# Avielstein/GRASP_LAB_SALP

Hardware: AMD Instinct MI355X
Metric: env-steps/sec at 65536 parallel envs, 1/2/4/8 MI355X; % HBM roofline (higher is better)
Workload: dtype f64

## Files before the change

grasp_lab_salp_amd/_codeobj.py:

```python
import hashlib
import struct

BUNDLE_MAGIC = b"__CLANG_OFFLOAD_BUNDLE__"


def _code_objects(blob):
    pos = 0
    while True:
        b = blob.find(BUNDLE_MAGIC, pos)
        if b < 0:
            return
        pos = b + len(BUNDLE_MAGIC)
        (n,) = struct.unpack_from("<Q", blob, pos)
        p = pos + 8
        for _ in range(n):
            off, size, idlen = struct.unpack_from("<QQQ", blob, p)
            p += 24
            ident = blob[p:p + idlen].decode("ascii", "replace")
            p += idlen
            if "amdgcn" in ident and size > 0:
                co = blob[b + off:b + off + size]
                if co[:4] == b"\x7fELF":
                    yield ident, co


def _symbols(co):
    shoff, = struct.unpack_from("<Q", co, 0x28)
    shentsize, shnum, _ = struct.unpack_from("<HHH", co, 0x3A)
    secs = []
    for k in range(shnum):
        (_name, sh_type, _flags, addr, off, size, link, _info, _align,
         entsize) = struct.unpack_from("<IIQQQQIIQQ", co, shoff + k * shentsize)
        secs.append((sh_type, addr, off, size, link, entsize))
    out = {}
    for sh_type, _addr, off, size, link, entsize in secs:
        if sh_type != 2:
            continue
        stroff = secs[link][2]
        for j in range(size // entsize):
            st_name, _st_info, _st_other, shndx, value, ssize = struct.unpack_from("<IBBHQQ", co, off + j * entsize)
            if shndx == 0 or shndx >= len(secs) or ssize == 0:
                continue
            end = co.index(b"\0", stroff + st_name)
            name = co[stroff + st_name:end].decode("ascii", "replace")
            s_addr, s_off = secs[shndx][1], secs[shndx][2]
            out[name] = (value - s_addr + s_off, ssize)
    return out


def kernel_symbols(lib_path, contains):
    blob = open(lib_path, "rb").read()
    names = set()
    for _ident, co in _code_objects(blob):
        syms = _symbols(co)
        names |= {n for n in syms if contains in n and n + ".kd" in syms}
    return sorted(names)


def _mask_layout(code):
    n = len(code) // 4
    w = list(struct.unpack("<%dI" % n, code[:4 * n]))
    for i in range(n):
        if (w[i] & 0xFF80FFFF) != 0xBE801C00:
            continue
        j = i + 1
        while j + 1 < n and j <= i + 4:
            op = w[j] & 0xFF800000
            lit = (w[j] & 0xFF) == 0xFF or (w[j] >> 8 & 0xFF) == 0xFF
            if op in (0x80000000, 0x82000000) and lit:
                w[j + 1] = 0
                j += 2
            else:
                j += 1
    return struct.pack("<%dI" % n, *w) + code[4 * n:]


def kernel_sha(lib_path, contains):
    blob = open(lib_path, "rb").read()
    for _ident, co in _code_objects(blob):
        syms = _symbols(co)
        hits = [n for n in syms if contains in n and n + ".kd" in syms]
        if len(hits) == 1:
            symbol = hits[0]
            h = hashlib.sha256()
            off, size = syms[symbol]
            h.update(_mask_layout(co[off:off + size]))
            off, size = syms[symbol + ".kd"]
            kd = bytearray(co[off:off + size])
            kd[16:24] = bytes(8)
            h.update(bytes(kd))
            return h.hexdigest()[:16]
    return None


ROLLOUT_KERNEL = "k_rolloutILb0ELb0EE"
PAIR_COLLECT_KERNEL = "k_rollout_pairILb1EE"
SPLIT_COLLECT_KERNEL = "k_rollout_splitILb1EE"


def collect_kernel():
    import os
    if (os.environ.get("SALP_TWO_WAVE_KERNEL") or "").startswith("p"):
        return PAIR_COLLECT_KERNEL, "k_rollout_pair<true>"
    return SPLIT_COLLECT_KERNEL, "k_rollout_split<true>"
```

grasp_lab_salp_amd/build.py:

```python
import argparse
import os
import subprocess
import sys

HERE = os.path.dirname(os.path.abspath(__file__))
SRCS = [os.path.join(HERE, "csrc", f) for f in ("salp_kernels.hip", "salp_gae.hip", "salp_ppo.hip", "salp_ppo_mlp.hip",
                                               "salp_sort.hip", "salp_lstm.hip", "salp_sac.hip")]
OUT = os.path.join(HERE, "libsalp.so")
ARCH = os.environ.get("SALP_OFFLOAD_ARCH", "gfx950")
HIPCC = os.environ.get("HIPCC", "/opt/rocm/bin/hipcc")

FLAGS = ["-O3", "-std=c++17", f"--offload-arch={ARCH}", "-ffp-contract=off", "-fno-fast-math",
         "-fPIC", "-shared", "-Wall", "-Wno-unused-function"]


def deps():
    c = os.path.join(HERE, "csrc")
    return SRCS + [os.path.join(c, f) for f in os.listdir(c) if f.endswith(".h")] + [
        os.path.join(HERE, "..", "include", "salp.h")]


def up_to_date():
    if not os.path.exists(OUT):
        return False
    t = os.path.getmtime(OUT)
    return all(os.path.getmtime(d) <= t for d in deps())


FILE_FLAGS = {"salp_ppo_mlp.hip": ["-mllvm", "-amdgpu-sched-strategy=max-ilp"]}


def build(force=False, verbose=False, extra=(), out=None, file_flags=None):
    if out is None and not force and up_to_date():
        return OUT
    out = out or OUT
    file_flags = FILE_FLAGS if file_flags is None else file_flags
    import tempfile
    from concurrent.futures import ThreadPoolExecutor
    compile_flags = [f for f in FLAGS if f != "-shared"]
    with tempfile.TemporaryDirectory(prefix="salp_build_") as tmp:
        objs = [os.path.join(tmp, os.path.basename(src) + ".o") for src in SRCS]
        cmds = [[HIPCC, *compile_flags, *file_flags.get(os.path.basename(src), []), *extra, "-c", "-o", obj, src]
                for src, obj in zip(SRCS, objs)]
        link = [HIPCC, f"--offload-arch={ARCH}", "-fPIC", "-shared", "-o", out + ".tmp", *objs]
        if verbose:
            for c in cmds + [link]:
                print(" ".join(c), flush=True)
        with ThreadPoolExecutor(max_workers=min(len(cmds), os.cpu_count() or 1)) as ex:
            for r in list(ex.map(lambda c: subprocess.run(c, capture_output=True, text=True), cmds)):
                if r.returncode:
                    raise subprocess.CalledProcessError(r.returncode, r.args, r.stdout, r.stderr)
                if r.stderr and verbose:
                    print(r.stderr, end="", flush=True)
        subprocess.run(link, check=True)
    os.replace(out + ".tmp", out)
    return out


if __name__ == "__main__":
    ap = argparse.ArgumentParser()
    ap.add_argument("--verbose", action="store_true")
    ap.add_argument("--force", action="store_true")
    ap.add_argument("--resource-usage", action="store_true")
    a = ap.parse_args()
    extra = ["-Rpass-analysis=kernel-resource-usage"] if a.resource_usage else []
    print(build(force=a.force or a.resource_usage, verbose=a.verbose, extra=extra))
    sys.exit(0)
```

grasp_lab_salp_amd/csrc/salp_kernels.hip:

```cpp
#include <hip/hip_runtime.h>

#include <cmath>
#include <cstdio>
#include <cstdlib>
#include <cstring>
#include <string>

#include "salp_device.h"
#include "salp_pair.h"
#include "salp_tanh.h"

using salp::Hot;
using salp::Params;

#define SF(f) salp::sref(S, P, i, (f))

namespace {

constexpr int kBlock = 256;
constexpr int kMaxTicksPerCycle = 1 << 16;
constexpr int64_t kSortMinEnvs = 1024;

static_assert(kBlock == salp::LANES, "LDS cache stride is the workgroup size");

// ... 236 lines not shown
    }
    if (reward_sum) reward_sum[i] = rs;
    salp::store_hot<RAND>(h, S, P, i);
}

__global__ __launch_bounds__(kBlock) void k_predict_ticks(const double* S, Params P, const float* actions,
                                                          int32_t n_steps, uint32_t* keys, int32_t* ids) {
    const int64_t i = (int64_t)blockIdx.x * blockDim.x + threadIdx.x;
    if (i >= P.n) return;
    double a1 = SF(SALP_F_ANGLE1), a2 = SF(SALP_F_ANGLE2);
    int64_t t = 0;
    if (actions) {
        t = salp::predict_cycle_ticks(P, actions[3 * i], actions[3 * i + 1], actions[3 * i + 2], &a1, &a2);
    } else {
        const uint64_t env_id = (uint64_t)(P.env_offset + i), sc = (uint64_t)SF(SALP_F_STEP_COUNT);
        for (int32_t k = 0; k < n_steps; ++k) {
            float a[3];
            sp_action(P.seed, env_id, sc + (uint64_t)k, a);
            t += salp::predict_cycle_ticks(P, a[0], a[1], a[2], &a1, &a2);
        }
    }
    keys[i] = (uint32_t)(t > 65535 ? 65535 : t);
    ids[i] = (int32_t)i;
}

constexpr int kPH = SALP_POLICY_HIDDEN, kPIN = SALP_OBS_DIM_MAX;
typedef const __attribute__((address_space(4))) float* PolicyW;

typedef float PolicyF2 __attribute__((ext_vector_type(2)));
static_assert(kPH % 2 == 0, "hidden units go in pairs");

__device__ __forceinline__ float policy_tanh(float x) { return salp_tanhf(x); }

__device__ __forceinline__ void policy_layer1(PolicyW w, int w1, int b1, const float* x, float* h1) {
#pragma unroll
    for (int j = 0; j < kPH; j += 2) {
        PolicyF2 acc = {w[b1 + j], w[b1 + j + 1]};
#pragma unroll
        for (int k = 0; k < kPIN; ++k) {
            const PolicyF2 wk = {w[w1 + j * kPIN + k], w[w1 + (j + 1) * kPIN + k]};
            const PolicyF2 xk = {x[k], x[k]};
            acc = __builtin_elementwise_fma(wk, xk, acc);
        }
        h1[j] = policy_tanh(acc.x);
        h1[j + 1] = policy_tanh(acc.y);
    }
}

template <int NOUT>
__device__ __forceinline__ void policy_mlp(PolicyW w, int w1, int b1, int w2, int b2, int hw,
                                           int hb, const float* x, float* out) {
    float h1[kPH];
    policy_layer1(w, w1, b1, x, h1);
#pragma unroll
    for (int c = 0; c < NOUT; ++c) out[c] = 0.0f;
#pragma unroll 1
    for (int j = 0; j < kPH; ++j) {
        PolicyF2 acc = {w[b2 + j], 0.0f};
#pragma unroll
        for (int k = 0; k < kPH; k += 2) {
            const PolicyF2 wk = {w[w2 + j * kPH + k], w[w2 + j * kPH + k + 1]};
            const PolicyF2 hk = {h1[k], h1[k + 1]};
            acc = __builtin_elementwise_fma(wk, hk, acc);
        }
        const float t = policy_tanh(acc.x + acc.y);
#pragma unroll
        for (int c = 0; c < NOUT; ++c) out[c] = fmaf(w[hw + c * kPH + j], t, out[c]);
    }
#pragma unroll
    for (int c = 0; c < NOUT; ++c) out[c] += w[hb + c];
}

constexpr int kPolL2 = kPH * kPH + kPH + 3 * kPH;
static_assert(SALP_POLICY_PI_B2 == SALP_POLICY_PI_W2 + kPH * kPH && SALP_POLICY_ACT_W == SALP_POLICY_PI_B2 + kPH,
              "the staged actor tensors are contiguous in the packed policy");
__device__ __forceinline__ void policy_actor_l2(PolicyW w, const float* l2, const float* x, float* out) {
    float h1[kPH];
    policy_layer1(w, SALP_POLICY_PI_W1, SALP_POLICY_PI_B1, x, h1);
    out[0] = out[1] = out[2] = 0.0f;
#pragma unroll 1
    for (int j = 0; j < kPH; ++j) {
        const float* row = l2 + j * kPH;
        PolicyF2 acc = {l2[kPH * kPH + j], 0.0f};
#pragma unroll
        for (int k = 0; k < kPH; k += 4) {
            const float4 v = *reinterpret_cast<const float4*>(row + k);
            acc = __builtin_elementwise_fma(PolicyF2{v.x, v.y}, PolicyF2{h1[k], h1[k + 1]}, acc);
            acc = __builtin_elementwise_fma(PolicyF2{v.z, v.w}, PolicyF2{h1[k + 2], h1[k + 3]}, acc);
        }
        const float t = policy_tanh(acc.x + acc.y);
#pragma unroll
        for (int c = 0; c < 3; ++c) out[c] = fmaf(l2[kPH * kPH + kPH + c * kPH + j], t, out[c]);
    }
#pragma unroll
    for (int c = 0; c < 3; ++c) out[c] += w[SALP_POLICY_ACT_B + c];
}

__device__ __forceinline__ void policy_input(const float* o, int obs_dim, float* x) {
#pragma unroll
    for (int k = 0; k < kPIN; ++k) x[k] = k < obs_dim ? o[k] : 0.0f;
}

__device__ __forceinline__ float policy_value(PolicyW w, const float* x) {
    float v;
    policy_mlp<1>(w, SALP_POLICY_VF_W1, SALP_POLICY_VF_B1, SALP_POLICY_VF_W2, SALP_POLICY_VF_B2, SALP_POLICY_VAL_W,
                  SALP_POLICY_VAL_B, x, &v);
    return v;
}

#define SP_STREAM_POLICY 7u
__device__ __forceinline__ void policy_noise(uint64_t seed, uint64_t env_id, uint64_t step, float z[3]) {
    const sp_u32x4 r = sp_draw(seed, env_id, step, SP_STREAM_POLICY, 0);
    const double u1 = ((double)r.v[0] + 1.0) * 0x1.0p-32, u3 = ((double)r.v[2] + 1.0) * 0x1.0p-32;
    const double rad1 = sqrt(-2.0 * sm_log(u1)), rad2 = sqrt(-2.0 * sm_log(u3));
    double s1, c1, s2, c2;
    sm_sincos(6.283185307179586 * sp_u01_32(r.v[1]), &s1, &c1);
    sm_sincos(6.283185307179586 * sp_u01_32(r.v[3]), &s2, &c2);
    z[0] = (float)(rad1 * c1);
    z[1] = (float)(rad1 * s1);
    z[2] = (float)(rad2 * c2);
}

template <bool L2 = false>
__device__ __forceinline__ void policy_act(const SalpPolicyRollout& R, int obs_dim, const float* o, uint64_t env_id,
                                           uint64_t step, float a[3], float* value, float* logp,
                                           const float* l2 = nullptr) {
    const PolicyW w = (PolicyW)R.weights;
    float x[kPIN];
    policy_input(o, obs_dim, x);
    float mean[3];
    if (L2)
        policy_actor_l2(w, l2, x, mean);
    else
        policy_mlp<3>(w, SALP_POLICY_PI_W1, SALP_POLICY_PI_B1, SALP_POLICY_PI_W2, SALP_POLICY_PI_B2,
                      SALP_POLICY_ACT_W, SALP_POLICY_ACT_B, x, mean);
    if (value) *value = policy_value(w, x);
    float z[3];
    policy_noise(R.noise_seed, env_id, step, z);
    float lp = 0.0f;
#pragma unroll
    for (int c = 0; c < 3; ++c) {
        const float ls = w[SALP_POLICY_LOG_STD + c], sd = expf(ls);
        a[c] = mean[c] + sd * z[c];
        const float d = a[c] - mean[c];
        lp += -(d * d) / (2.0f * (sd * sd)) - logf(sd) - 0.91893853320467274f;
    }
    *logp = lp;
}

struct ValuesInPlace {
    static constexpr bool kDefer = false;
    static constexpr bool kL2 = false;
    __device__ __forceinline__ const float* l2() const { return nullptr; }
    __device__ __forceinline__ void start_rep() {}
    __device__ __forceinline__ void boot(const float*, int, float, int64_t) {}
    __device__ __forceinline__ void value(const float*, int, int64_t) {}
    __device__ __forceinline__ void publish() {}
};

#ifndef SALP_COLLECT_REP_MIN
#define SALP_COLLECT_REP_MIN 4
#endif

__device__ __forceinline__ float clamp_box(float a, float lo, float hi) { return a < lo ? lo : (a > hi ? hi : a); }

template <bool RAND, bool POL, class ST, class VS = ValuesInPlace>
__device__ __forceinline__ void rollout_boundary(Hot& h, ST S, const Params& P, int64_t i,
                                                 uint64_t env_id, bool& pending, bool& active,
                                                 int64_t& steps, int64_t max_steps,
                                                 const SalpRolloutBuffers& B, double* reward_sum,
                                                 const SalpPolicyRollout& R, salp::Cache32 c32, VS vs = VS()) {
    float o[SALP_OBS_DIM_MAX];
    bool have_o = false;
    float ep_start = 0.0f;
    for (int rep = 0; rep < 4; ++rep) {
        const bool fin = active && pending && !(h.ct < h.b2);
        vs.start_rep();
        if (fin) {
            SF(SALP_F_STEP_COUNT) = SF(SALP_F_STEP_COUNT) + 1.0;
            salp::StepOut r = salp::finish_step<RAND>(h, S, P, i, o, nullptr);
            bool reset = r.terminated || r.truncated;
            if (POL) {
                const size_t row = (size_t)steps * (size_t)P.n + (size_t)i;
                float rew = (float)r.reward;
                bool bad = false;
                if (R.diverged_obs_abs > 0.0) {
                    bad = !(fabs(r.reward) <= R.diverged_reward_abs);
                    for (int k = 0; k < P.obs_dim; ++k) bad = bad || !(fabsf(o[k]) <= (float)R.diverged_obs_abs);
                }
                if (bad) {
                    rew = 0.0f;
                    atomicAdd((unsigned long long*)R.diverged, 1ull);
                } else if (r.truncated && !r.terminated) {
                    if (VS::kDefer) {
                        vs.boot(o, P.obs_dim, rew, (int64_t)steps);
                    } else {
                        float x[kPIN];
                        policy_input(o, P.obs_dim, x);
                        rew = rew + (float)R.gamma * policy_value((PolicyW)R.weights, x);
                    }
                }
                if (reset && !bad) {
                    atomicAdd(&R.ep_stats[0], SF(SALP_F_EP_RETURN));
                    atomicAdd(&R.ep_stats[1], 1.0);
                    if (r.terminated) atomicAdd(&R.ep_stats[2], 1.0);
                    atomicAdd(&R.ep_stats[3], SF(SALP_F_EP_LEN));
                }
                if (!(VS::kDefer && !bad && r.truncated && !r.terminated)) R.rewards[row] = rew;
                reset = reset || bad;
                ep_start = reset ? 1.0f : 0.0f;
                R.episode_start[i] = ep_start;
            } else if (B.capacity > 0) {
                const size_t slot = (size_t)(steps % B.capacity);
                const size_t row = slot * (size_t)P.n + (size_t)i;
                if (B.obs)
                    for (int k = 0; k < P.obs_dim; ++k) B.obs[row * P.obs_dim + k] = o[k];
                if (B.actions) {
                    B.actions[row * 3 + 0] = (float)SF(SALP_F_ACT0);
                    B.actions[row * 3 + 1] = (float)SF(SALP_F_ACT1);
                    B.actions[row * 3 + 2] = (float)SF(SALP_F_ACT2);
                }
                if (B.rewards) B.rewards[row] = (float)r.reward;
                if (B.dones) B.dones[row] = (uint8_t)((r.terminated ? 1 : 0) | (r.truncated ? 2 : 0));
            }
            if (reward_sum) reward_sum[i] += r.reward;
            ++steps;
            pending = false;
            if (reset) salp::reset_env_philox(h, S, P, i, (POL || B.obs_before) ? o : nullptr);
            have_o = true;
            if (max_steps > 0 && steps >= max_steps) {
                active = false;
                if (POL)
                    for (int k = 0; k < P.obs_dim; ++k) R.last_obs[(size_t)i * P.obs_dim + k] = o[k];
            }
        }
        const bool beg = active && !pending;
        if (beg) {
            if (POL && !have_o) {
                for (int k = 0; k < P.obs_dim; ++k) o[k] = R.last_obs[(size_t)i * P.obs_dim + k];
                have_o = true;
            } else if (B.obs_before && !have_o) {
                const salp::Rot Rt = salp::rot_zyx(h.e0, h.e1, h.e2);
                salp::observation(h, Rt, S, P, i, o);
                have_o = true;
            }
            if (POL && VS::kDefer) vs.value(o, P.obs_dim, (int64_t)steps);
        }
        vs.publish();
        if (beg) {
            float a[3];
            if (POL) {
                if (!fin) ep_start = R.episode_start[i];
                float raw[3], v, lp;
                policy_act<VS::kL2>(R, P.obs_dim, o, env_id, (uint64_t)SF(SALP_F_STEP_COUNT), raw,
                                    VS::kDefer ? nullptr : &v, &lp, vs.l2());
                const size_t row = (size_t)steps * (size_t)P.n + (size_t)i;
                for (int k = 0; k < P.obs_dim; ++k) R.obs[row * P.obs_dim + k] = o[k];
                R.actions[row * 3 + 0] = raw[0];
                R.actions[row * 3 + 1] = raw[1];
                R.actions[row * 3 + 2] = raw[2];
                if (!VS::kDefer) R.values[row] = v;
                R.log_probs[row] = lp;
                R.episode_starts[row] = ep_start;
                a[0] = clamp_box(raw[0], 0.0f, 1.0f);
                a[1] = clamp_box(raw[1], 0.0f, 1.0f);
                a[2] = clamp_box(raw[2], -1.0f, 1.0f);
            } else {
                if (B.obs_before && B.capacity > 0) {
                    const size_t row = (size_t)(steps % B.capacity) * (size_t)P.n + (size_t)i;
                    for (int k = 0; k < P.obs_dim; ++k) B.obs_before[row * P.obs_dim + k] = o[k];
                }
                sp_action(P.seed, env_id, (uint64_t)SF(SALP_F_STEP_COUNT), a);
            }
            salp::begin_step<RAND>(h, S, P, i, a[0], a[1], a[2], c32);
            pending = true;
        }
        if (POL && SALP_COLLECT_REP_MIN > 1) {
            const bool again = active && pending && !(h.ct < h.b2);
            if (__popcll(__ballot(again)) < SALP_COLLECT_REP_MIN) break;
        }
        if (VS::kDefer) {
            if (!__any(fin || beg)) break;
        } else if (!fin && !beg) {
            break;
        }
    }
}

struct RolloutArgs {
    double* S;
    Params P;
    int64_t n_chunks;
    int32_t chunk;
    int32_t steady_q8;
    int64_t max_steps;
    SalpRolloutBuffers B;
    double* reward_sum;
    int32_t fresh;
    int32_t pad_;
    SalpPolicyRollout R;
};
static_assert(sizeof(RolloutArgs) % 8 == 0, "RolloutArgs is copied as 8-byte words");
typedef const __attribute__((address_space(4))) uint64_t* KernargWords;
__device__ __forceinline__ RolloutArgs fresh_args() {
    KernargWords p = (KernargWords)__builtin_amdgcn_kernarg_segment_ptr();
    asm volatile("" : "+s"(p));
    uint64_t w[sizeof(RolloutArgs) / 8];
    for (size_t k = 0; k < sizeof(RolloutArgs) / 8; ++k) w[k] = p[k];
    RolloutArgs a;
    __builtin_memcpy(&a, w, sizeof a);
    return a;
}

#ifndef SALP_ROLLOUT_RESEAT
#define SALP_ROLLOUT_RESEAT 1
#endif

__device__ __forceinline__ int nth_set_lane(const uint64_t* m, int k) {
    constexpr int NW = kBlock / 64;
    int base = 0;
    uint64_t w = m[NW - 1];
#pragma unroll
    for (int j = 0; j < NW - 1; ++j) {
        const int c = __popcll(m[j]);
        if (k < c) {
            w = m[j];
            base = 64 * j;
            break;
        }
        k -= c;
        base = 64 * (j + 1);
    }
    int pos = 0;
#pragma unroll
    for (int half = 32; half > 0; half >>= 1) {
        const uint64_t lo = w & ((1ull << half) - 1ull);
        const int c = __popcll(lo);
        if (k >= c) {
            k -= c;
            w >>= half;
            pos += half;
        } else {
            w = lo;
        }
    }
    return base + pos;
}

__device__ __forceinline__ bool unsteady(const Hot& h, const Params& P, bool active) {
    return active && h.ct < h.b2 && !salp::next_tick_steady(h, P);
}

template <bool RAND, bool POL>
__device__ __forceinline__ bool lane_boundary(const RolloutArgs& a, salp::SpillSlot sp, int64_t i, bool& pending,
                                              bool& active, int64_t& steps, double* c32p) {
    const uint64_t env_id = (uint64_t)(a.P.env_offset + i);
    salp::ColdRegs<RAND> C;
    salp::load_cold<RAND>(C, a.S, a.P, i);
    Hot hb;
    salp::unspill<RAND>(hb, sp, a.P, env_id);
    rollout_boundary<RAND, POL>(hb, &C, a.P, i, env_id, pending, active, steps, a.max_steps, a.B,
                                a.reward_sum, a.R, salp::Cache32{c32p});
    salp::store_cold<RAND>(C, a.S, a.P, i);
    salp::spill<RAND>(hb, sp);
    return unsteady(hb, a.P, active);
}
template <bool RAND, bool POL>
__device__ __noinline__ bool lane_boundary_call(const RolloutArgs* a, double* spp, int64_t i, bool* pending,
                                                bool* active, int64_t* steps, double* c32p) {
    return lane_boundary<RAND, POL>(*a, salp::SpillSlot{spp}, i, *pending, *active, *steps, c32p);
}

#ifndef SALP_ROLLOUT_PROF
#define SALP_ROLLOUT_PROF 0
#endif
enum { RP_BOUNDARY, RP_FULL, RP_STEADY, RP_SETTLED, RP_BARRIER, RP_RESEAT, RP_N };
__device__ unsigned long long g_roll_prof[2][RP_N];
struct RollProf {
    unsigned long long cyc[RP_N] = {}, its[RP_N] = {};
    unsigned long long t = 0;
    __device__ __forceinline__ void start() {
        if (SALP_ROLLOUT_PROF) t = __builtin_amdgcn_s_memtime();
    }
    __device__ __forceinline__ void lap(int part, int64_t iterations = 0) {
        if (SALP_ROLLOUT_PROF) {
            const unsigned long long now = __builtin_amdgcn_s_memtime();
            cyc[part] += now - t;
            its[part] += (unsigned long long)iterations;
            t = now;
        }
    }
    __device__ __forceinline__ void flush() {
        if (SALP_ROLLOUT_PROF && (threadIdx.x & 63) == 0)
            for (int k = 0; k < RP_N; ++k) {
                atomicAdd(&g_roll_prof[0][k], cyc[k]);
                atomicAdd(&g_roll_prof[1][k], its[k]);
            }
    }
};

#if SALP_ROLLOUT_RESEAT
template <bool RAND, bool POL>
__global__ __launch_bounds__(kBlock) void k_rollout(RolloutArgs A) {
    double* const S = A.S;
    const Params& P = A.P;
    const int64_t base = (int64_t)blockIdx.x * blockDim.x;
    const int lane = (int)threadIdx.x;
    __shared__ double s_cache32[salp::C32_N * salp::LANES];
    __shared__ double s_spill[salp::SPILL_N * salp::LANES];
    __shared__ int64_t s_steps[kBlock];
    __shared__ uint8_t s_flags[kBlock];
    __shared__ int16_t s_slot[2][kBlock];
    __shared__ uint64_t s_mask[2][kBlock / 64];
    __shared__ uint64_t s_amask[2][kBlock / 64];
    int s = lane;
    int64_t i = base + s;
    bool pending = false, active = false;
    int64_t steps = 0;
    Hot h{};
    if (i < P.n) {
        pending = !A.fresh && SF(SALP_F_PENDING) != 0.0;
        steps = A.B.steps_done ? A.B.steps_done[i] : 0;
        active = !(A.max_steps > 0 && steps >= A.max_steps);
        salp::load_hot<RAND>(h, S, P, i);
        salp::resume_cycle(h, S, P, i);
        salp::fill_cache32(P, h.c, salp::Cache32{s_cache32 + s});
    }
    if (!active) h.b2 = -INFINITY;
    bool all_done = false;
    RollProf prof;
    prof.start();
    for (int64_t c = 0;; ++c) {
        const bool last = c == A.n_chunks || all_done;
        const salp::SpillSlot sp{s_spill + s};
        const bool need = active && (!pending || !(h.ct < h.b2));
        bool uns = unsteady(h, P, active);
        salp::spill<RAND>(h, sp);
        if (need) {
            if (RAND) {
                uns = lane_boundary_call<RAND, POL>(&A, s_spill + s, i, &pending, &active, &steps, s_cache32 + s);
            } else {
                const RolloutArgs a = fresh_args();
                uns = lane_boundary<RAND, POL>(a, sp, i, pending, active, steps, s_cache32 + s);
            }
        }
        if (last) {
            const RolloutArgs a = fresh_args();
            salp::unspill<RAND>(h, sp, a.P, (uint64_t)(a.P.env_offset + i));
            if (i < a.P.n) salp::store_hot<RAND>(h, a.S, a.P, i);
            break;
        }
        const int b = (int)(c & 1);
        s_steps[s] = steps;
        s_flags[s] = (uint8_t)((pending ? 1 : 0) | (active ? 2 : 0));
        s_slot[b][lane] = (int16_t)s;
        const uint64_t ballot = __ballot(uns);
        const uint64_t aballot = __ballot(active);
        if ((lane & 63) == 0) {
            s_mask[b][lane >> 6] = ballot;
            s_amask[b][lane >> 6] = aballot;
        }
        prof.lap(RP_BOUNDARY);
        __syncthreads();
        prof.lap(RP_BARRIER);
        uint64_t m[kBlock / 64];
        int n_uns = 0;
        uint64_t any_active = 0;
#pragma unroll
        for (int w = 0; w < kBlock / 64; ++w) {
            m[w] = s_mask[b][w];
            n_uns += __popcll(m[w]);
            any_active |= s_amask[b][w];
        }
        all_done = any_active == 0;
        int from;
        if (lane < n_uns) {
            from = nth_set_lane(m, lane);
        } else {
#pragma unroll
            for (int w = 0; w < kBlock / 64; ++w) m[w] = ~m[w];
            from = nth_set_lane(m, lane - n_uns);
        }
        s = s_slot[b][from];
        i = base + s;
        const int fl = s_flags[s];
        pending = (fl & 1) != 0;
        active = (fl & 2) != 0;
        steps = s_steps[s];
        {
            const RolloutArgs a = fresh_args();
            salp::unspill<RAND>(h, salp::SpillSlot{s_spill + s}, a.P, (uint64_t)(a.P.env_offset + i));
        }
        if (!active) h.b2 = -INFINITY;
        if (all_done) continue;
        prof.lap(RP_RESEAT);
        const salp::Cache32 c32{s_cache32 + s};
        const Params PV = salp::pin_params(P);
        int32_t k = 0;
        for (; k < A.chunk; ++k) {
            if (__all(!(h.ct < h.b2) || salp::next_tick_steady(h, PV))) break;
            if (h.ct < h.b2) salp::tick<false, RAND, true>(h, PV, c32);
        }
        prof.lap(RP_FULL, k);
        const int32_t ks = (int32_t)(((int64_t)(A.chunk - k) * A.steady_q8) >> 8);
        int32_t j = 0;
        for (; j < ks; ++j) {
            bool settled = true;
            if (h.ct < h.b2) settled = salp::tick<false, RAND, true, true>(h, PV, c32);
            if (__all(settled)) {
                ++j;
                break;
            }
        }
        prof.lap(RP_STEADY, j);
        const int32_t j0 = j;
        for (; j < ks; ++j)
            if (h.ct < h.b2) salp::tick<false, RAND, true, true, true>(h, PV, c32);
        prof.lap(RP_SETTLED, j - j0);
    }
    prof.flush();
    if (A.B.steps_done && i < P.n) A.B.steps_done[i] = steps;
}
#else
template <bool RAND, bool POL>
__global__ __launch_bounds__(kBlock) void k_rollout(RolloutArgs A) {
    double* const S = A.S;
    const Params& P = A.P;
    int64_t i = (int64_t)blockIdx.x * blockDim.x + threadIdx.x;
    if (i >= P.n) return;
    bool pending = !A.fresh && SF(SALP_F_PENDING) != 0.0;
    int64_t steps = A.B.steps_done ? A.B.steps_done[i] : 0;
    bool active = !(A.max_steps > 0 && steps >= A.max_steps);
    LANE_CACHE32();
    __shared__ double s_spill[salp::SPILL_N * salp::LANES];
    const salp::SpillSlot sp{s_spill + threadIdx.x};
    Hot h;
    salp::load_hot<RAND>(h, S, P, i);
    salp::resume_cycle(h, S, P, i);
    salp::fill_cache32(P, h.c, c32);
    if (!active) h.b2 = -INFINITY;
    for (int64_t c = 0; c <= A.n_chunks; ++c) {
        const bool need = active && (!pending || !(h.ct < h.b2));
        const bool last = c == A.n_chunks || !__any(active || need);
        if (__any(need) || last) {
            salp::spill<RAND>(h, sp);
            if (need) {
                const RolloutArgs a = fresh_args();
                const uint64_t env_id = (uint64_t)(a.P.env_offset + i);
                salp::ColdRegs<RAND> C;
                salp::load_cold<RAND>(C, a.S, a.P, i);
                Hot hb;
                salp::unspill<RAND>(hb, sp, a.P, env_id);
                rollout_boundary<RAND, POL>(hb, &C, a.P, i, env_id, pending, active, steps, a.max_steps, a.B,
                                            a.reward_sum, a.R, c32);
                salp::store_cold<RAND>(C, a.S, a.P, i);
                salp::spill<RAND>(hb, sp);
            }
            {
                const RolloutArgs a = fresh_args();
                salp::unspill<RAND>(h, sp, a.P, (uint64_t)(a.P.env_offset + i));
                if (last) {
                    salp::store_hot<RAND>(h, a.S, a.P, i);
                    break;
                }
            }
            if (!active) h.b2 = -INFINITY;
        }
        const Params PV = salp::pin_params(P);
        for (int32_t k = 0; k < A.chunk; ++k)
            if (h.ct < h.b2) salp::tick<false, RAND, true>(h, PV, c32);
    }
    if (A.B.steps_done) A.B.steps_done[i] = steps;
}
#endif

constexpr int kPairEnvs = 128;
constexpr int kXchAB = 5;
constexpr int kXchBA = 13;
constexpr int kXchBase = 4 * kXchAB * 64;
constexpr int kXchDoubles = kXchBase + 4 * kXchBA * 64;
static_assert(kXchDoubles <= salp::SPILL_N * kPairEnvs, "the packets live in the spill slots' LDS");
constexpr int kPairSpin = 1 << 21;
__device__ unsigned int g_pair_timeouts;

#ifndef SALP_PAIR_PROF
#define SALP_PAIR_PROF 0
#endif
enum { PP_BOUNDARY, PP_TICK, PP_PUBLISH, PP_WAIT, PP_READ, PP_WORLD, PP_BARRIER, PP_N };
__device__ unsigned long long g_pair_prof[2][PP_N];
struct PairProf {
    unsigned long long acc[PP_N] = {};
    unsigned long long t = 0;
    __device__ __forceinline__ void start() {
        if (SALP_PAIR_PROF) t = __builtin_amdgcn_s_memtime();
    }
    __device__ __forceinline__ void lap(int phase) {
        if (SALP_PAIR_PROF) {
            const unsigned long long now = __builtin_amdgcn_s_memtime();
            acc[phase] += now - t;
            t = now;
        }
    }
    __device__ __forceinline__ void flush(int role) {
        if (SALP_PAIR_PROF && (threadIdx.x & 63) == 0)
            for (int k = 0; k < PP_N; ++k) atomicAdd(&g_pair_prof[role][k], acc[k]);
    }
};

struct PairShared {
    double cache32[salp::C32_N * kPairEnvs];
    double big[salp::SPILL_N * kPairEnvs];
    int64_t steps[kPairEnvs];
    int16_t slot[2][kPairEnvs];
    uint64_t mask[2][2], amask[2][2];
    int cnt[2][2];
    int mode[2][2];
    uint8_t flags[kPairEnvs];
};

struct PairJobs {
    __attribute__((aligned(16))) float pi_l2[kPolL2];
    float boot_obs[4][kPIN][kPairEnvs];
    float val_obs[4][kPIN][kPairEnvs];
    float boot_rew[4][kPairEnvs];
    int32_t boot_step[4][kPairEnvs];
    int32_t val_step[4][kPairEnvs];
    uint8_t flags[4][kPairEnvs];
    int cnt[2];
    int done[2];
};

__device__ __forceinline__ bool pair_wait(int* flag, int target) {
    for (int it = 0; it < kPairSpin; ++it) {
        if (__hip_atomic_load(flag, __ATOMIC_ACQUIRE, __HIP_MEMORY_SCOPE_WORKGROUP) >= target) return true;
        __builtin_amdgcn_s_sleep(1);
    }
    if ((threadIdx.x & 63) == 0) atomicAdd(&g_pair_timeouts, 1u);
    return false;
}
__device__ __forceinline__ void pair_publish(int* flag, int value) {
    __hip_atomic_store(flag, value, __ATOMIC_RELEASE, __HIP_MEMORY_SCOPE_WORKGROUP);
}

constexpr int kWaveRing = 64;
enum { WR_V0, WR_V1, WR_V2, WR_W0, WR_W1, WR_W2, WR_STRIDE = 6 };
enum { WX_E0, WX_E1, WX_E2, WX_P0, WX_P1, WX_P2, WX_SP, WX_CP, WX_ST, WX_CTH, WX_FAIL, WX_N };
struct WaveShared {
    double rows[kWave * WG_STRIDE];
    double ring[kWaveRing * WR_STRIDE];
    double xchg[WX_N];
    double c32[salp::C32_N];
    int produced, consumed;
};

template <bool RAND>
__device__ __forceinline__ bool run_cycle_split(Hot& h, const Params& P, salp::Cache32 c32, WaveShared& W) {
    const bool kin = threadIdx.x >= kWave;
    bool ok = true;
    int g = 0;
    if (!kin) {
        while (h.ct < h.b2 && g < kMaxTicksPerCycle) {
            wave_geometry_rows(h, P, c32, W.rows);
            __builtin_amdgcn_fence(__ATOMIC_ACQ_REL, "workgroup");
            int last = 0;
            for (int j = 0; j < kWave && h.ct < h.b2 && g < kMaxTicksPerCycle; ++j, ++g) {
                double x[WG_RI1 + 1];
                const double* r = W.rows + j * WG_STRIDE;
#pragma unroll
                for (int k = 0; k <= WG_RI1; ++k) x[k] = r[k];
                const bool settled = h.phase != salp::JET &&
                                     (__double_as_longlong(h.geo.mr) | __double_as_longlong(h.comr) |
                                      __double_as_longlong(h.coma)) == 0 &&
                                     h.geo.I0 == h.pI0 && h.geo.I1 == h.pI1 && h.pI2 == h.pI1;
                if (settled)
                    salp::tick_dynamics<false, RAND, true, salp::TD_FORCES | salp::TD_POSITIONS>(h, P, nullptr, 0);
                else
                    salp::tick_dynamics<false, RAND, false, salp::TD_FORCES | salp::TD_POSITIONS>(h, P, nullptr, 0);
                if (g >= kWaveRing) ok = pair_wait(&W.consumed, g - kWaveRing + 1) && ok;
                double* q = W.ring + (g % kWaveRing) * WR_STRIDE;
                q[WR_V0] = h.v0; q[WR_V1] = h.v1; q[WR_V2] = h.v2;
                q[WR_W0] = h.w0; q[WR_W1] = h.w1; q[WR_W2] = h.w2;
                pair_publish(&W.produced, g + 1);
                h.ct = x[WG_CT]; h.time = x[WG_TIME]; h.phase = (int)x[WG_PHASE]; h.W = x[WG_W];
                h.com = x[WG_COM]; h.comr = x[WG_COMR]; h.coma = x[WG_COMA];
                salp::Geo& q2 = h.geo;
                q2.m = x[WG_M]; q2.mr = x[WG_MR]; q2.I0 = x[WG_I0]; q2.I1 = x[WG_I1];
                q2.kc0 = x[WG_KC0]; q2.kc1 = x[WG_KC1]; q2.ra0 = x[WG_RA0]; q2.ra1 = x[WG_RA1];
                q2.dimx = x[WG_DIMX]; q2.dimy = x[WG_DIMY]; q2.speed = x[WG_SPEED]; q2.rx = x[WG_RX];
                q2.rm = x[WG_RM]; q2.rI0 = x[WG_RI0]; q2.rI1 = x[WG_RI1];
                last = j;
            }
            const double* r = W.rows + last * WG_STRIDE;
            h.L = r[WG_L]; h.V = r[WG_V]; h.pV = r[WG_PV];
            h.g32 = r[WG_G32] != 0.0; h.pv32 = r[WG_PV32] != 0.0;
            __builtin_amdgcn_fence(__ATOMIC_ACQ_REL, "workgroup");
        }
    } else {
        double ct = h.ct;
        for (; ct < h.b2 && g < kMaxTicksPerCycle; ++g) {
            ok = pair_wait(&W.produced, g + 1) && ok;
            const double* q = W.ring + (g % kWaveRing) * WR_STRIDE;
            h.v0 = q[WR_V0]; h.v1 = q[WR_V1]; h.v2 = q[WR_V2];
            h.w0 = q[WR_W0]; h.w1 = q[WR_W1]; h.w2 = q[WR_W2];
            pair_publish(&W.consumed, g + 1);
            salp::tick_dynamics<false, RAND, false, salp::TD_KINEMATICS>(h, P, nullptr, 0);
            ct += salp::DT;
        }
    }
    return ok;
}

template <bool RAND>
__global__ __launch_bounds__(2 * kWave) void k_step_wave(double* S, Params P, const float* actions,
                                                         float* obs_out, double* reward_out,
                                                         uint8_t* term_out, uint8_t* trunc_out,
                                                         int auto_reset, float* term_obs_out, double* info_out) {
    const int64_t i = blockIdx.x;
    if (i >= P.n) return;
    __shared__ __attribute__((aligned(16))) WaveShared W;
    const salp::Cache32 c32{W.c32, 1};
    const bool kin = threadIdx.x >= kWave;
    if (threadIdx.x == 0) {
        W.produced = 0;
        W.consumed = 0;
    }
    Hot h;
    salp::load_hot<RAND>(h, S, P, i);
    {
        salp::ColdRegs<RAND> C;
        salp::load_cold<RAND>(C, S, P, i);
        salp::begin_step<RAND>(h, &C, P, i, actions[3 * i], actions[3 * i + 1], actions[3 * i + 2], c32);
        if (!kin) salp::store_cold<RAND>(C, S, P, i);
    }
    __syncthreads();
    const bool ok = run_cycle_split<RAND>(h, P, c32, W);
    __syncthreads();
    if (kin) {
        if (threadIdx.x == kWave) {
            double* x = W.xchg;
            x[WX_E0] = h.e0; x[WX_E1] = h.e1; x[WX_E2] = h.e2;
            x[WX_P0] = h.p0; x[WX_P1] = h.p1; x[WX_P2] = h.p2;
            x[WX_SP] = h.sp; x[WX_CP] = h.cp; x[WX_ST] = h.st; x[WX_CTH] = h.cth;
            x[WX_FAIL] = ok ? 0.0 : 1.0;
        }
    }
    __syncthreads();
    if (kin) return;
    {
        const double* x = W.xchg;
        h.e0 = x[WX_E0]; h.e1 = x[WX_E1]; h.e2 = x[WX_E2];
        h.p0 = x[WX_P0]; h.p1 = x[WX_P1]; h.p2 = x[WX_P2];
        h.sp = x[WX_SP]; h.cp = x[WX_CP]; h.st = x[WX_ST]; h.cth = x[WX_CTH];
        if (!ok || x[WX_FAIL] != 0.0) salp::poison_motion(h);
    }
    float o[SALP_OBS_DIM_MAX];
    double* info = info_out ? info_out + (size_t)SALP_INFO_DIM * i : nullptr;
    salp::ColdRegs<RAND> C;
    salp::load_cold<RAND>(C, S, P, i);
    double& sc = salp::sref(&C, P, i, SALP_F_STEP_COUNT);
    sc = sc + 1.0;
    const salp::StepOut r = salp::finish_step<RAND>(h, &C, P, i, o, info);
    if (term_obs_out)
        for (int k = 0; k < P.obs_dim; ++k) term_obs_out[(size_t)i * P.obs_dim + k] = o[k];
    if (auto_reset && (r.terminated || r.truncated)) salp::reset_env_philox(h, &C, P, i, o);
    salp::store_cold<RAND>(C, S, P, i);
    if (reward_out) reward_out[i] = r.reward;
    if (term_out) term_out[i] = r.terminated;
    if (trunc_out) trunc_out[i] = r.truncated;
    if (obs_out)
        for (int k = 0; k < P.obs_dim; ++k) obs_out[(size_t)i * P.obs_dim + k] = o[k];
    salp::store_hot<RAND>(h, S, P, i);
}

struct ValuesToPartner {
    static constexpr bool kDefer = true;
    static constexpr bool kL2 = true;
    PairJobs* J;
    int grp, s, buf;
    __device__ __forceinline__ const float* l2() const { return J->pi_l2; }
    __device__ __forceinline__ void start_rep() {
        buf = __hip_atomic_load(&J->cnt[grp], __ATOMIC_RELAXED, __HIP_MEMORY_SCOPE_WORKGROUP) & 3;
    }
    __device__ __forceinline__ void boot(const float* o, int od, float rew, int64_t step) {
        for (int k = 0; k < od; ++k) J->boot_obs[buf][k][s] = o[k];
        J->boot_rew[buf][s] = rew;
        J->boot_step[buf][s] = (int32_t)step;
        J->flags[buf][s] |= 1;
    }
    __device__ __forceinline__ void value(const float* o, int od, int64_t step) {
        for (int k = 0; k < od; ++k) J->val_obs[buf][k][s] = o[k];
        J->val_step[buf][s] = (int32_t)step;
        J->flags[buf][s] |= 2;
    }
    __device__ __forceinline__ void publish() {
        const int c = __hip_atomic_load(&J->cnt[grp], __ATOMIC_RELAXED, __HIP_MEMORY_SCOPE_WORKGROUP);
        pair_publish(&J->cnt[grp], c + 1);
    }
};

__device__ __forceinline__ void pair_value_jobs(PairJobs& J, const RolloutArgs& A, int grp, int s, int64_t c,
                                                int& taken) {
    const PolicyW w = (PolicyW)A.R.weights;
    const int64_t i = (int64_t)blockIdx.x * kPairEnvs + s;
    const int od = A.P.obs_dim;
    for (int it = 0; it < kPairSpin; ++it) {
        const int pub = __hip_atomic_load(&J.cnt[grp], __ATOMIC_ACQUIRE, __HIP_MEMORY_SCOPE_WORKGROUP);
        if (taken < pub) {
            const int b = taken & 3;
            const int f = J.flags[b][s];
            if (f & 1) {
                float x[kPIN];
#pragma unroll
                for (int k = 0; k < kPIN; ++k) x[k] = k < od ? J.boot_obs[b][k][s] : 0.0f;
                const float rew = J.boot_rew[b][s] + (float)A.R.gamma * policy_value(w, x);
                A.R.rewards[(size_t)J.boot_step[b][s] * (size_t)A.P.n + (size_t)i] = rew;
            }
            if (f & 2) {
                float x[kPIN];
#pragma unroll
                for (int k = 0; k < kPIN; ++k) x[k] = k < od ? J.val_obs[b][k][s] : 0.0f;
                A.R.values[(size_t)J.val_step[b][s] * (size_t)A.P.n + (size_t)i] = policy_value(w, x);
// ... 1395 lines not shown
```

Before: 70.18 million.

## Outline reseat rollout tick loop into noinline wave_ticks function

Moves the per-chunk tick loops of the reseat rollout kernel into a separate noinline device function. The function reloads kernel args from the kernarg pointer and unspills and respills the hot state from LDS, so the main kernel carries only a flags word across boundaries instead of the full Hot state. The aim is to cut register pressure in the kernel body, giving better allocation or occupancy, at the cost of call overhead and the extra spill and unspill traffic. The code-object hashing now also covers callee functions so the fingerprint tracks the outlined code.

```diff
diff --git a/grasp_lab_salp_amd/_codeobj.py b/grasp_lab_salp_amd/_codeobj.py
--- a/grasp_lab_salp_amd/_codeobj.py
+++ b/grasp_lab_salp_amd/_codeobj.py
@@ -24,7 +24,7 @@
                     yield ident, co
 
 
-def _symbols(co):
+def _symtab(co):
     shoff, = struct.unpack_from("<Q", co, 0x28)
     shentsize, shnum, _ = struct.unpack_from("<HHH", co, 0x3A)
     secs = []
@@ -32,20 +32,25 @@
         (_name, sh_type, _flags, addr, off, size, link, _info, _align,
          entsize) = struct.unpack_from("<IIQQQQIIQQ", co, shoff + k * shentsize)
         secs.append((sh_type, addr, off, size, link, entsize))
-    out = {}
     for sh_type, _addr, off, size, link, entsize in secs:
         if sh_type != 2:
             continue
         stroff = secs[link][2]
         for j in range(size // entsize):
-            st_name, _st_info, _st_other, shndx, value, ssize = struct.unpack_from("<IBBHQQ", co, off + j * entsize)
+            st_name, st_info, _st_other, shndx, value, ssize = struct.unpack_from("<IBBHQQ", co, off + j * entsize)
             if shndx == 0 or shndx >= len(secs) or ssize == 0:
                 continue
             end = co.index(b"\0", stroff + st_name)
             name = co[stroff + st_name:end].decode("ascii", "replace")
-            s_addr, s_off = secs[shndx][1], secs[shndx][2]
-            out[name] = (value - s_addr + s_off, ssize)
-    return out
+            yield name, st_info, value, value - secs[shndx][1] + secs[shndx][2], ssize
+
+
+def _symbols(co):
+    return {name: (off, size) for name, _info, _addr, off, size in _symtab(co)}
+
+
+def _functions(co):
+    return {addr: (name, off, size) for name, info, addr, off, size in _symtab(co) if (info & 0xF) == 2}
 
 
 def kernel_symbols(lib_path, contains):
@@ -75,6 +80,35 @@
     return struct.pack("<%dI" % n, *w) + code[4 * n:]
 
 
+def _pc_relative_targets(code, address):
+    n = len(code) // 4
+    w = struct.unpack("<%dI" % n, code[:4 * n])
+    out = []
+    for i in range(n):
+        if (w[i] & 0xFF80FFFF) != 0xBE801C00:
+            continue
+        for j in range(i + 1, min(i + 5, n - 1)):
+            if (w[j] & 0xFF800000) == 0x80000000 and ((w[j] & 0xFF) == 0xFF or (w[j] >> 8 & 0xFF) == 0xFF):
+                lit = w[j + 1] - (1 << 32) if w[j + 1] & 0x80000000 else w[j + 1]
+                out.append(address + 4 * (i + 1) + lit)
+                break
+    return out
+
+
+def _callees(co, address, funcs):
+    seen, out = {address}, []
+
+    def visit(addr):
+        _name, off, size = funcs[addr]
+        for t in _pc_relative_targets(co[off:off + size], addr):
+            if t in funcs and t not in seen:
+                seen.add(t)
+                out.append(funcs[t])
+                visit(t)
+    visit(address)
+    return out
+
+
 def kernel_sha(lib_path, contains):
     blob = open(lib_path, "rb").read()
     for _ident, co in _code_objects(blob):
@@ -89,6 +123,11 @@
             kd = bytearray(co[off:off + size])
             kd[16:24] = bytes(8)
             h.update(bytes(kd))
+            funcs = _functions(co)
+            entry = [a for a, (n, _o, _s) in funcs.items() if n == symbol]
+            for name, off, size in (_callees(co, entry[0], funcs) if entry else []):
+                h.update(b"\0callee\0")
+                h.update(_mask_layout(co[off:off + size]))
             return h.hexdigest()[:16]
     return None
 
diff --git a/grasp_lab_salp_amd/build.py b/grasp_lab_salp_amd/build.py
--- a/grasp_lab_salp_amd/build.py
+++ b/grasp_lab_salp_amd/build.py
@@ -17,7 +17,7 @@
 def deps():
     c = os.path.join(HERE, "csrc")
     return SRCS + [os.path.join(c, f) for f in os.listdir(c) if f.endswith(".h")] + [
-        os.path.join(HERE, "..", "include", "salp.h")]
+        os.path.join(HERE, "..", "include", "salp.h"), os.path.abspath(__file__)]
 
 
 def up_to_date():
diff --git a/grasp_lab_salp_amd/csrc/salp_kernels.hip b/grasp_lab_salp_amd/csrc/salp_kernels.hip
--- a/grasp_lab_salp_amd/csrc/salp_kernels.hip
+++ b/grasp_lab_salp_amd/csrc/salp_kernels.hip
@@ -562,14 +562,16 @@
 };
 static_assert(sizeof(RolloutArgs) % 8 == 0, "RolloutArgs is copied as 8-byte words");
 typedef const __attribute__((address_space(4))) uint64_t* KernargWords;
-__device__ __forceinline__ RolloutArgs fresh_args() {
-    KernargWords p = (KernargWords)__builtin_amdgcn_kernarg_segment_ptr();
+__device__ __forceinline__ RolloutArgs args_at(KernargWords p) {
     asm volatile("" : "+s"(p));
     uint64_t w[sizeof(RolloutArgs) / 8];
     for (size_t k = 0; k < sizeof(RolloutArgs) / 8; ++k) w[k] = p[k];
     RolloutArgs a;
     __builtin_memcpy(&a, w, sizeof a);
     return a;
+}
+__device__ __forceinline__ RolloutArgs fresh_args() {
+    return args_at((KernargWords)__builtin_amdgcn_kernarg_segment_ptr());
 }
 
 #ifndef SALP_ROLLOUT_RESEAT
@@ -660,6 +662,62 @@
 };
 
 #if SALP_ROLLOUT_RESEAT
+typedef __attribute__((address_space(3))) double LdsDouble;
+enum { TK_TICKING = 1, TK_UNSTEADY = 2 };
+__device__ __forceinline__ RolloutArgs args_of(uint64_t kernarg) {
+    const uint32_t lo = __builtin_amdgcn_readfirstlane((uint32_t)kernarg);
+    const uint32_t hi = __builtin_amdgcn_readfirstlane((uint32_t)(kernarg >> 32));
+    return args_at((KernargWords)(((uint64_t)hi << 32) | lo));
+}
+__device__ __forceinline__ uint32_t tick_flags(const Hot& h, const Params& P, bool active) {
+    return (uint32_t)((h.ct < h.b2 ? TK_TICKING : 0) | (unsteady(h, P, active) ? TK_UNSTEADY : 0));
+}
+#if SALP_ROLLOUT_PROF
+#define ROLL_PROF_PARAM , RollProf& prof
+#define ROLL_PROF_ARG , prof
+#else
+#define ROLL_PROF_PARAM
+#define ROLL_PROF_ARG
+#endif
+template <bool RAND>
+__device__ __noinline__ uint32_t wave_ticks(uint64_t kernarg, LdsDouble* spp, LdsDouble* c32p, int64_t i,
+                                            uint32_t active ROLL_PROF_PARAM) {
+#if !SALP_ROLLOUT_PROF
+    RollProf prof;
+#endif
+    const salp::SpillSlot sp{(double*)spp};
+    const salp::Cache32 c32{(double*)c32p};
+    const RolloutArgs A = args_of(kernarg);
+    const int32_t chunk = A.chunk, steady_q8 = A.steady_q8;
+    Hot h;
+    salp::unspill<RAND>(h, sp, A.P, (uint64_t)(A.P.env_offset + i));
+    if (!active) h.b2 = -INFINITY;
+    prof.lap(RP_RESEAT);
+    const Params PV = salp::pin_params(A.P);
+    int32_t k = 0;
+    for (; k < chunk; ++k) {
+        if (__all(!(h.ct < h.b2) || salp::next_tick_steady(h, PV))) break;
+        if (h.ct < h.b2) salp::tick<false, RAND, true>(h, PV, c32);
+    }
+    prof.lap(RP_FULL, k);
+    const int32_t ks = (int32_t)(((int64_t)(chunk - k) * steady_q8) >> 8);
+    int32_t j = 0;
+    while (j < ks) {
+        bool settled = true;
+        if (h.ct < h.b2) settled = salp::tick<false, RAND, true, true>(h, PV, c32);
+        ++j;
+        if (__all(settled)) break;
+    }
+    prof.lap(RP_STEADY, j);
+    const int32_t j0 = j;
+    for (; j < ks; ++j)
+        if (h.ct < h.b2) salp::tick<false, RAND, true, true, true>(h, PV, c32);
+    prof.lap(RP_SETTLED, j - j0);
+    const uint32_t tk = tick_flags(h, args_of(kernarg).P, active != 0);
+    salp::spill<RAND>(h, sp);
+    return tk;
+}
+
 template <bool RAND, bool POL>
 __global__ __launch_bounds__(kBlock) void k_rollout(RolloutArgs A) {
     double* const S = A.S;
@@ -677,25 +735,29 @@
     int64_t i = base + s;
     bool pending = false, active = false;
     int64_t steps = 0;
-    Hot h{};
-    if (i < P.n) {
-        pending = !A.fresh && SF(SALP_F_PENDING) != 0.0;
-        steps = A.B.steps_done ? A.B.steps_done[i] : 0;
-        active = !(A.max_steps > 0 && steps >= A.max_steps);
-        salp::load_hot<RAND>(h, S, P, i);
-        salp::resume_cycle(h, S, P, i);
-        salp::fill_cache32(P, h.c, salp::Cache32{s_cache32 + s});
-    }
-    if (!active) h.b2 = -INFINITY;
+    uint32_t tk;
+    {
+        Hot h{};
+        if (i < P.n) {
+            pending = !A.fresh && SF(SALP_F_PENDING) != 0.0;
+            steps = A.B.steps_done ? A.B.steps_done[i] : 0;
+            active = !(A.max_steps > 0 && steps >= A.max_steps);
+            salp::load_hot<RAND>(h, S, P, i);
+            salp::resume_cycle(h, S, P, i);
+            salp::fill_cache32(P, h.c, salp::Cache32{s_cache32 + s});
+        }
+        if (!active) h.b2 = -INFINITY;
+        tk = tick_flags(h, P, active);
+        salp::spill<RAND>(h, salp::SpillSlot{s_spill + s});
+    }
     bool all_done = false;
     RollProf prof;
     prof.start();
     for (int64_t c = 0;; ++c) {
         const bool last = c == A.n_chunks || all_done;
         const salp::SpillSlot sp{s_spill + s};
-        const bool need = active && (!pending || !(h.ct < h.b2));
-        bool uns = unsteady(h, P, active);
-        salp::spill<RAND>(h, sp);
+        const bool need = active && (!pending || !(tk & TK_TICKING));
+        bool uns = (tk & TK_UNSTEADY) != 0;
         if (need) {
             if (RAND) {
                 uns = lane_boundary_call<RAND, POL>(&A, s_spill + s, i, &pending, &active, &steps, s_cache32 + s);
@@ -706,6 +768,7 @@
         }
         if (last) {
             const RolloutArgs a = fresh_args();
+            Hot h;
             salp::unspill<RAND>(h, sp, a.P, (uint64_t)(a.P.env_offset + i));
             if (i < a.P.n) salp::store_hot<RAND>(h, a.S, a.P, i);
             break;
@@ -747,36 +810,9 @@
         pending = (fl & 1) != 0;
         active = (fl & 2) != 0;
         steps = s_steps[s];
-        {
-            const RolloutArgs a = fresh_args();
-            salp::unspill<RAND>(h, salp::SpillSlot{s_spill + s}, a.P, (uint64_t)(a.P.env_offset + i));
-        }
-        if (!active) h.b2 = -INFINITY;
         if (all_done) continue;
-        prof.lap(RP_RESEAT);
-        const salp::Cache32 c32{s_cache32 + s};
-        const Params PV = salp::pin_params(P);
-        int32_t k = 0;
-        for (; k < A.chunk; ++k) {
-            if (__all(!(h.ct < h.b2) || salp::next_tick_steady(h, PV))) break;
-            if (h.ct < h.b2) salp::tick<false, RAND, true>(h, PV, c32);
-        }
-        prof.lap(RP_FULL, k);
-        const int32_t ks = (int32_t)(((int64_t)(A.chunk - k) * A.steady_q8) >> 8);
-        int32_t j = 0;
-        for (; j < ks; ++j) {
-            bool settled = true;
-            if (h.ct < h.b2) settled = salp::tick<false, RAND, true, true>(h, PV, c32);
-            if (__all(settled)) {
-                ++j;
-                break;
-            }
-        }
-        prof.lap(RP_STEADY, j);
-        const int32_t j0 = j;
-        for (; j < ks; ++j)
-            if (h.ct < h.b2) salp::tick<false, RAND, true, true, true>(h, PV, c32);
-        prof.lap(RP_SETTLED, j - j0);
+        tk = wave_ticks<RAND>((uint64_t)__builtin_amdgcn_kernarg_segment_ptr(), (LdsDouble*)(s_spill + s),
+                              (LdsDouble*)(s_cache32 + s), i, active ? 1u : 0u ROLL_PROF_ARG);
     }
     prof.flush();
     if (A.B.steps_done && i < P.n) A.B.steps_done[i] = steps;
```

Measured after the change: 72.68 million (median of 6 runs). 3.6% higher.
